# hrnr/map-merge

Hardware: NVIDIA B200
Metric: pairwise_registrations_per_sec (higher is better)
Workload: dtype f32

## Files before the change

map-merge_b200/csrc/icp.cu:

```cuda
#include <algorithm>
#include <cmath>
#include <cstring>
#include <type_traits>

#include "mm3d_internal.cuh"

namespace mm3d {

namespace {

constexpr int IB = 128;
constexpr int NSUM = 17;

struct IcpState {
  float final_t[16];
  float step[16];
  double prev_mse;
  int iterations;
  int active;
  int converged;
  int pad;
};

struct IcpJob {
  GridView tgt;
  ReachView reach;
  const float4* src;
  int ns;
  float4* work;
  long long* sums;
  IcpState* st;
  int* ticket;
  int* next_tile;
  int n_tiles;
  float t0[16];
  long long* sums_log;
  int* nn_slot;
};

struct IcpLoop {
  int n_active;
  int pad[3];
};

struct ReachJob {
  GridView g;
  ReachView r;
  unsigned char* a;
  unsigned char* b;
};

__global__ void __launch_bounds__(256) reach_mark_kernel(const ReachJob* __restrict__ jobs)
{
  const ReachJob& j = jobs[blockIdx.y];
  for (int i = blockIdx.x * blockDim.x + threadIdx.x; i < j.g.n; i += gridDim.x * blockDim.x) {
    const float4 p = j.g.pts[i];
    const int x = floor_to_int(p.x * j.g.inv_leaf) - j.g.min_b[0] - j.r.org[0];
    const int y = floor_to_int(p.y * j.g.inv_leaf) - j.g.min_b[1] - j.r.org[1];
    const int z = floor_to_int(p.z * j.g.inv_leaf) - j.g.min_b[2] - j.r.org[2];
    if (x >= 0 && y >= 0 && z >= 0 && x < j.r.dim[0] && y < j.r.dim[1] && z < j.r.dim[2])
      j.a[((size_t)z * j.r.dim[1] + y) * j.r.dim[0] + x] = 0;
  }
}

__global__ void __launch_bounds__(256) reach_pass_kernel(const ReachJob* __restrict__ jobs, int axis, int margin, int from_a)
{
// ... 9 lines not shown
    const int len = j.r.dim[axis];
    const long long stride = axis == 0 ? 1 : (axis == 1 ? (long long)j.r.dim[0] : (long long)j.r.dim[0] * j.r.dim[1]);
    const int lo = max(-margin, -pos), hi = min(margin, len - 1 - pos);
    int best = 255;
    for (int d = lo; d <= hi; ++d) {
      const int f = max(abs(d) - 1, 0);
      const int v = (int)in[(long long)c + (long long)d * stride] + f * f;
      best = min(best, v);
    }
    out[c] = (unsigned char)min(best, j.r.none);
  }
}

__device__ __forceinline__ bool reach_lookup(const GridView& g, const ReachView& r, float qx, float qy, float qz, int* lb2)
{
  const int x = floor_to_int(qx * g.inv_leaf) - g.min_b[0] - r.org[0];
  const int y = floor_to_int(qy * g.inv_leaf) - g.min_b[1] - r.org[1];
  const int z = floor_to_int(qz * g.inv_leaf) - g.min_b[2] - r.org[2];
  if (x < 0 || y < 0 || z < 0 || x >= r.dim[0] || y >= r.dim[1] || z >= r.dim[2]) return false;
  *lb2 = (int)__ldg(&r.lb2[((size_t)z * r.dim[1] + y) * r.dim[0] + x]);
  return true;
}

__device__ __forceinline__ bool reach_descend(const ReachView& r, int& x, int& y, int& z, int cur)
{
  for (int step = 0; step < 48 && cur > 0; ++step) {
    int best = cur, bx = x, by = y, bz = z;
#pragma unroll
    for (int t = 0; t < 6; ++t) {
      const int nx = x + (t == 0) - (t == 1), ny = y + (t == 2) - (t == 3), nz = z + (t == 4) - (t == 5);
      if (nx < 0 || ny < 0 || nz < 0 || nx >= r.dim[0] || ny >= r.dim[1] || nz >= r.dim[2]) continue;
      const int v = (int)__ldg(&r.lb2[((size_t)nz * r.dim[1] + ny) * r.dim[0] + nx]);
      if (v < best) {
        best = v;
        bx = nx;
        by = ny;
        bz = nz;
      }
    }
    if (best >= cur) return false;
    cur = best;
    x = bx;
    y = by;
    z = bz;
  }
  return cur == 0;
}

__device__ __forceinline__ float block27_any(const GridView& g, int vx, int vy, int vz, float qx, float qy, float qz)
// ... 62 lines not shown
    for (int k = rs[t]; k < re[t]; ++k) {
      const float4 p = g.pts[k];
      const float d2 = em::dist2_3(qx, qy, qz, p.x, p.y, p.z);
      if ((double)d2 > bound) continue;
      const int oi = g.orig ? g.orig[k] : k;
      if (!found || d2 < best || (d2 == best && oi < best_idx)) {
        found = true;
        best = d2;
        best_idx = oi;
        best_slot = k;
        best_pt = p;
        bestv = d2 * inv2 * 1.0001f + 1e-4f;
      }
    }
  }
  *certain = found && best * inv2 < 0.999f;
  *out_idx = best_idx;
  *out_d2 = best;
  *out_pt = best_pt;
  *out_slot = found ? best_slot : -1;
  return found;
}

struct TileNn {
  float4 q[IB];
  int todo[IB];
  int todo_large[IB];
  float res_d2[IB];
  int res_slot[IB];
  int n_todo, n_todo_large;
};

__device__ __forceinline__ bool tile_nearest(TileNn& sh, const GridView& g, const ReachView& r, bool live, float qx, float qy, float qz,
                                             double bound, int guess_slot, float* out_d2, float4* out_pt, int* out_slot)
{
  const int tid = threadIdx.x, lane = tid & 31, warp = tid >> 5;
  if (tid == 0) {
    sh.n_todo = 0;
    sh.n_todo_large = 0;
  }
  __syncthreads();
  bool hit = false, pending = false;
  float d2 = 0.f;
  int slot = -1;
  float4 pt = make_float4(0.f, 0.f, 0.f, 0.f);
  if (live) {
    float r2 = (float)bound;
    bool rejected = false, block_has_points = true;
    if (r.lb2) {
      int lb2 = 0;
      const float bound_v = (float)bound * g.inv_leaf * g.inv_leaf;
      const bool inside = reach_lookup(g, r, qx, qy, qz, &lb2);
      const float lb = inside ? (float)lb2 : (float)r.none;
      if (lb > bound_v * 1.001f + 0.01f) rejected = true;
      if (inside && lb2 < r.none) {
        const float ub = sqrtf((float)lb2) + 3.4642f;
        r2 = fminf(r2, (ub * ub * 1.001f + 0.01f) * g.leaf * g.leaf);
      }
      block_has_points = inside && lb2 == 0;
      if (!rejected && inside && lb2 > 0 && lb2 < r.none && guess_slot < 0 && g.shift[0] == 0 && g.shift[1] == 0 && g.shift[2] == 0) {
        int cx = floor_to_int(qx * g.inv_leaf) - g.min_b[0] - r.org[0];
        int cy = floor_to_int(qy * g.inv_leaf) - g.min_b[1] - r.org[1];
        int cz = floor_to_int(qz * g.inv_leaf) - g.min_b[2] - r.org[2];
        if (reach_descend(r, cx, cy, cz, lb2)) {
          const float dd = block27_any(g, cx + r.org[0], cy + r.org[1], cz + r.org[2], qx, qy, qz);
          if (dd < 3.0e38f) r2 = fminf(r2, dd);
        }
      }
    }
    if (!rejected) {
      bool certain = false;
      if ((block_has_points || guess_slot >= 0) && g.shift[0] == 0 && g.shift[1] == 0 && g.shift[2] == 0) {
        int idx;
        hit = nearest_block27(g, qx, qy, qz, bound, guess_slot, &idx, &d2, &pt, &slot, &certain);
        if (hit) r2 = fminf(r2, d2);
      }
      if (!certain) {
        pending = true;
        hit = false;
        const float r2w = r2 * 1.00001f + 1e-12f;
        sh.q[tid] = make_float4(qx, qy, qz, r2w);
        if (r2w * g.inv_leaf * g.inv_leaf <= 12.25f) sh.todo[atomicAdd(&sh.n_todo, 1)] = tid;
        else sh.todo_large[atomicAdd(&sh.n_todo_large, 1)] = tid;
      }
    }
  }
  __syncthreads();
  const int n_small = sh.n_todo, n_large = sh.n_todo_large;
  auto serve = [&](auto G_, int who, unsigned gmask, int glane) {
    constexpr int G = decltype(G_)::value;
    const float4 q = sh.q[who];
    const int rv = (int)ceilf(sqrtf(q.w) * g.inv_leaf) + 1;
    float bd = 3.0e38f;
    int bi = 0x7fffffff, bs = -1;
    group_radius_unordered<G>(g, gmask, glane, q.x, q.y, q.z, q.w, rv, [&](bool valid, int k, const float4&, float dd) {
      if (valid && (double)dd <= bound) {
        const int oi = g.orig ? g.orig[k] : k;
        if (dd < bd || (dd == bd && oi < bi)) {
          bd = dd;
          bi = oi;
          bs = k;
        }
      }
    });
#pragma unroll
    for (int o = G / 2; o > 0; o >>= 1) {
      const float od = __shfl_xor_sync(gmask, bd, o, G);
      const int oi = __shfl_xor_sync(gmask, bi, o, G);
      const int os = __shfl_xor_sync(gmask, bs, o, G);
      if (od < bd || (od == bd && oi < bi)) {
        bd = od;
        bi = oi;
        bs = os;
      }
    }
    if (glane == 0) {
      sh.res_d2[who] = bd;
      sh.res_slot[who] = bs;
    }
  };
  {
    const int grp = tid >> 3, glane = tid & 7;
    const unsigned gmask = 0xffu << (lane & 24);
    for (int t = grp; t < n_small; t += IB / 8) serve(std::integral_constant<int, 8>(), sh.todo[t], gmask, glane);
  }
  __syncwarp();
  for (int t = warp; t < n_large; t += IB / 32) serve(std::integral_constant<int, 32>(), sh.todo_large[t], 0xffffffffu, lane);
  __syncthreads();
  if (pending) {
    slot = sh.res_slot[tid];
    hit = slot >= 0;
    if (hit) {
      d2 = sh.res_d2[tid];
      pt = g.pts[slot];
    }
  }
  *out_d2 = d2;
  *out_pt = pt;
  *out_slot = hit ? slot : -1;
  return hit;
}

__global__ void __launch_bounds__(256) icp_init_kernel(const IcpJob* __restrict__ jobs)
{
  const IcpJob& j = jobs[blockIdx.y];
  for (int i = blockIdx.x * blockDim.x + threadIdx.x; i < j.ns; i += gridDim.x * blockDim.x) {
    const float4 p = j.src[i];
    float4 o;
    em::transform_point(j.t0, p.x, p.y, p.z, &o.x, &o.y, &o.z);
    o.w = p.w;
    j.work[i] = o;
    j.nn_slot[i] = -1;
  }
}

__device__ __forceinline__ void block_accumulate(long long* vals, int nvals, long long* gsums)
{
  __shared__ long long sh[IB / 32][NSUM];
  const int lane = threadIdx.x & 31, w = threadIdx.x >> 5;
  __syncthreads();
  for (int k = 0; k < nvals; ++k) {
    const long long v = warp_sum_ll(vals[k]);
    if (lane == 0) sh[w][k] = v;
  }
  __syncthreads();
  if (threadIdx.x < nvals) {
    long long s = 0;
    for (int ww = 0; ww < IB / 32; ++ww) s += sh[ww][threadIdx.x];
    if (s != 0) atomicAdd((unsigned long long*)&gsums[threadIdx.x], (unsigned long long)s);
  }
}

__device__ void mat4_mul(const float* a, const float* b, float* r)
{
  for (int i = 0; i < 4; ++i)
    for (int c = 0; c < 4; ++c) {
      float acc = a[i * 4 + 0] * b[0 * 4 + c];
      acc += a[i * 4 + 1] * b[1 * 4 + c];
      acc += a[i * 4 + 2] * b[2 * 4 + c];
      acc += a[i * 4 + 3] * b[3 * 4 + c];
      r[i * 4 + c] = acc;
    }
}

__device__ void icp_solve(const IcpJob& j, int max_iterations, double rotation_threshold, double translation_threshold, int max_log,
                          int* n_active)
{
  IcpState& st = *j.st;
  long long s[NSUM];
  for (int k = 0; k < NSUM; ++k) {
    s[k] = (long long)atomicExch((unsigned long long*)&j.sums[k], 0ull);
  }
  if (j.sums_log && st.iterations < max_log)
// ... 27 lines not shown
    st.step[k] = T[k];
  }
  st.iterations += 1;
  bool conv = false;
  if (st.iterations >= max_iterations) {
    conv = true;
  } else {
    const double cos_angle = 0.5 * (double)(T[0] + T[5] + T[10] - 1);
    const double translation_sqr = (double)(T[3] * T[3] + T[7] * T[7] + T[11] * T[11]);
    if (cos_angle >= rotation_threshold && translation_sqr <= translation_threshold) {
      conv = true;
    } else {
      const double mse = ((double)s[16] / MM3D_FIXD_SCALE) / n;
      if (fabs(mse - st.prev_mse) < 1e-12) conv = true;
      else st.prev_mse = mse;
    }
  }
  if (conv) {
    st.active = 0;
    st.converged = 1;
    __threadfence();
    atomicSub(n_active, 1);
  } else {
    __threadfence();
    atomicExch(j.next_tile, 0);
  }
}

__device__ __forceinline__ void icp_tile(const IcpJob& j, int tile, double max_dist_sqr, int rv, int max_iterations,
                                         double rotation_threshold, double translation_threshold, int max_log, int* n_active)
{
  __shared__ float s_step[16];
  __shared__ int s_apply;
  __shared__ TileNn nn;
  __syncthreads();
  if (threadIdx.x < 16) s_step[threadIdx.x] = __ldcg(&j.st->step[threadIdx.x]);
  if (threadIdx.x == 16) s_apply = __ldcg(&j.st->iterations) > 0 ? 1 : 0;
  __syncthreads();
  const int apply_step = s_apply;
  long long v[NSUM];
#pragma unroll
  for (int k = 0; k < NSUM; ++k) v[k] = 0;
  const int i = tile * IB + threadIdx.x;
  const bool live = i < j.ns;
  float4 p = make_float4(0.f, 0.f, 0.f, 0.f);
  int guess = -1;
  if (live) {
    p = __ldcg(&j.work[i]);
    if (apply_step) {
      float4 o;
      em::transform_point(s_step, p.x, p.y, p.z, &o.x, &o.y, &o.z);
      o.w = p.w;
      p = o;
      j.work[i] = p;
    }
    guess = __ldcg(&j.nn_slot[i]);
  }
  float d2;
  float4 q;
  int slot;
  const bool hit = tile_nearest(nn, j.tgt, j.reach, live, p.x, p.y, p.z, max_dist_sqr, guess, &d2, &q, &slot);
  if (live) {
    j.nn_slot[i] = slot;
    if (hit) {
      const double pp[3] = {(double)p.x, (double)p.y, (double)p.z};
      const double qq[3] = {(double)q.x, (double)q.y, (double)q.z};
      v[0] = 1;
#pragma unroll
      for (int a = 0; a < 3; ++a) {
        v[1 + a] = em::to_fix(pp[a], MM3D_FIX1_SCALE);
        v[4 + a] = em::to_fix(qq[a], MM3D_FIX1_SCALE);
#pragma unroll
        for (int b = 0; b < 3; ++b) v[7 + a * 3 + b] = em::to_fix(qq[a] * pp[b], MM3D_FIX2_SCALE);
      }
      v[16] = em::to_fix((double)d2, MM3D_FIXD_SCALE);
    }
  }
  block_accumulate(v, NSUM, j.sums);
  __syncthreads();
  if (threadIdx.x == 0) {
    __threadfence();
    const int ntiles = (j.ns + IB - 1) / IB;
    const int ticket = atomicAdd(j.ticket, 1);
    if (ticket == ntiles - 1) {
      *j.ticket = 0;
      __threadfence();
      icp_solve(j, max_iterations, rotation_threshold, translation_threshold, max_log, n_active);
    }
  }
}

__global__ void __launch_bounds__(IB) icp_persistent_kernel(const IcpJob* __restrict__ jobs, int n_jobs, IcpLoop* loop, double max_dist_sqr,
                                                            int rv, int max_iterations, double rotation_threshold,
                                                            double translation_threshold, int max_log)
{
  __shared__ int s_pair, s_tile;
  int cur = 0;
  for (;;) {
    if (threadIdx.x == 0) {
      int pair = -1, tile = -1, scanned = 0;
      while (__ldcg(&loop->n_active) > 0) {
        const IcpJob& j = jobs[cur];
        if (__ldcg(j.next_tile) < j.n_tiles) {
          const int t = atomicAdd(j.next_tile, 1);
          if (t < j.n_tiles) {
            __threadfence();
            pair = cur;
            tile = t;
            break;
          }
        }
        cur = cur + 1 == n_jobs ? 0 : cur + 1;
        if (++scanned >= n_jobs) {
          scanned = 0;
          __nanosleep(500);
        }
      }
      s_pair = pair;
      s_tile = tile;
    }
    __syncthreads();
    const int pair = s_pair, tile = s_tile;
    if (pair < 0) break;
    icp_tile(jobs[pair], tile, max_dist_sqr, rv, max_iterations, rotation_threshold, translation_threshold, max_log, &loop->n_active);
    __syncthreads();
  }
}

struct ScoreJob {
  GridView tgt;
  ReachView reach;
  const float4* src;
  int ns;
  float t[16];
  long long* sums;
  const int* nn_guess;
};

__global__ void __launch_bounds__(IB) score_kernel(const ScoreJob* __restrict__ jobs, double max_range, int rv)
{
  const ScoreJob& j = jobs[blockIdx.y];
  if (blockIdx.x * IB >= j.ns) return;
  __shared__ TileNn nn;
  long long v[2] = {0, 0};
  const int i = blockIdx.x * IB + threadIdx.x;
  const bool live = i < j.ns;
  float x = 0.f, y = 0.f, z = 0.f;
  if (live) {
    const float4 p = j.src[i];
    em::transform_point(j.t, p.x, p.y, p.z, &x, &y, &z);
  }
  float d2;
  float4 q;
  int slot;
  if (tile_nearest(nn, j.tgt, j.reach, live, x, y, z, max_range, (live && j.nn_guess) ? j.nn_guess[i] : -1, &d2, &q, &slot)) {
    v[0] = em::to_fix((double)d2, MM3D_FIXD_SCALE);
    v[1] = 1;
  }
  block_accumulate(v, 2, j.sums);
}

ReachView no_reach()
{
  ReachView r;
  memset(&r, 0, sizeof(r));
  return r;
}

}

void build_reach_batch(Ctx& c, const std::vector<DIndex>& idx, int margin, std::vector<DReach>& out)
{
  const int M = (int)idx.size();
  out.clear();
  out.resize(M);
  margin = std::max(2, std::min(margin, 15));
  std::vector<ReachJob> jobs;
  std::vector<DBuf<unsigned char>> ping(M);
  size_t max_cells = 0;
  int max_n = 0;
  for (int m = 0; m < M; ++m) {
    out[m].v = no_reach();
// ... 50 lines not shown
    if (zero) {
      for (int k = 0; k < 16; ++k) out[p].T[k] = 0.0f;
      out[p].iterations = 0;
      out[p].converged = 0;
    } else {
      act.push_back(p);
    }
  }
  const int A = (int)act.size();
  if (A == 0) return;
  std::stable_sort(act.begin(), act.end(), [&](int x, int y) { return jobs[x].b < jobs[y].b; });
  size_t tot = 0;
  int mx = 0;
  for (int a = 0; a < A; ++a) {
    tot += (size_t)clouds[jobs[act[a]].a].n;
    mx = std::max(mx, clouds[jobs[act[a]].a].n);
  }
  DBuf<float4> work(c, tot + 1);
  DBuf<int> nn_local;
  DBuf<int>& nn = nn_keep ? nn_keep->slots : nn_local;
  nn.alloc(c, tot + 1);
  DBuf<long long> sums(c, (size_t)A * NSUM);
  sums.zero(c);
  DBuf<int> tickets(c, A);
  tickets.zero(c);
  DBuf<long long> slog;
  if (max_log) {
    slog.alloc(c, (size_t)A * max_log * NSUM);
    slog.zero(c);
  }
  std::vector<IcpState> hst(A);
  for (int a = 0; a < A; ++a) {
    memset(&hst[a], 0, sizeof(IcpState));
    for (int k = 0; k < 16; ++k) hst[a].final_t[k] = hst[a].step[k] = (k % 5 == 0) ? 1.f : 0.f;
    hst[a].prev_mse = 1.7976931348623157e308;
    hst[a].active = clouds[jobs[act[a]].a].n > 0 ? 1 : 0;
  }
  DBuf<IcpState> dst = to_device(c, hst);
  std::vector<IcpJob> ij(A);
  size_t off = 0;
  for (int a = 0; a < A; ++a) {
    const PairJob& pj = jobs[act[a]];
    ij[a].tgt = idx[pj.b].v;
    ij[a].reach = pj.b < (int)reach.size() ? reach[pj.b].v : no_reach();
    ij[a].src = clouds[pj.a].pts;
    ij[a].ns = clouds[pj.a].n;
    ij[a].work = work.p + off;
    ij[a].nn_slot = nn.p + off;
    if (nn_keep) nn_keep->offset[act[a]] = (long long)off;
    ij[a].sums = sums.p + (size_t)a * NSUM;
    ij[a].st = dst.p + a;
    ij[a].ticket = tickets.p + a;
    for (int k = 0; k < 16; ++k) ij[a].t0[k] = T0[act[a]][k];
    ij[a].sums_log = max_log ? slog.p + (size_t)a * max_log * NSUM : nullptr;
    off += (size_t)ij[a].ns;
  }
  std::vector<int> hnext(A, 0);
  IcpLoop hl;
  memset(&hl, 0, sizeof(hl));
  int tiles = 0;
  double bytes = 0;
  for (int a = 0; a < A; ++a) {
    ij[a].n_tiles = (ij[a].ns + IB - 1) / IB;
    if (hst[a].active) {
      hl.n_active += 1;
      tiles += ij[a].n_tiles;
      bytes += 16.0 * (2.0 * ij[a].ns + ij[a].tgt.n);
    } else {
      hnext[a] = ij[a].n_tiles;
    }
  }
  DBuf<int> dnext = to_device(c, hnext);
  for (int a = 0; a < A; ++a) ij[a].next_tile = dnext.p + a;
  DBuf<IcpJob> dij = to_device(c, ij);
  DBuf<IcpLoop> dloop(c, 1);
  dloop.upload(c, &hl, 1);
  const int iblocks = std::max(1, std::min((mx + 255) / 256, 148 * 8));
  MM_LAUNCH(c, icp_init_kernel, dim3(iblocks, A), 256, 0, dij.p);
  const double max_dist_sqr = max_dist * max_dist;
  const float leaf = idx[jobs[act[0]].b].v.leaf;
  const int rv = (int)std::ceil(max_dist / (double)leaf) + 1;
  if (hl.n_active > 0) {
    int dev = 0, sms = 0, per_sm = 0;
    MM_CUDA(cudaGetDevice(&dev));
    MM_CUDA(cudaDeviceGetAttribute(&sms, cudaDevAttrMultiProcessorCount, dev));
    MM_CUDA(cudaOccupancyMaxActiveBlocksPerMultiprocessor(&per_sm, icp_persistent_kernel, IB, 0));
    const int grid = std::max(1, std::min(sms * std::max(per_sm, 1), tiles));
    MM_BYTES(c, bytes);
    MM_LAUNCH(c, icp_persistent_kernel, grid, IB, 0, dij.p, A, dloop.p, max_dist_sqr, rv, max_it, 1.0 - eps, eps, max_log);
  }
  dst.download(c, hst.data(), A);
  std::vector<long long> hlog;
  if (max_log) {
    hlog.resize((size_t)A * max_log * NSUM);
    slog.download(c, hlog.data(), hlog.size());
  }
  c.sync();
  for (int a = 0; a < A; ++a) {
    IcpOut& o = out[act[a]];
    const float* f = hst[a].final_t;
    const float* g = T0[act[a]];
    for (int i = 0; i < 4; ++i)
      for (int cc = 0; cc < 4; ++cc) {
        float acc = f[i * 4 + 0] * g[0 * 4 + cc];
        acc += f[i * 4 + 1] * g[1 * 4 + cc];
        acc += f[i * 4 + 2] * g[2 * 4 + cc];
        acc += f[i * 4 + 3] * g[3 * 4 + cc];
        o.T[i * 4 + cc] = acc;
      }
    o.iterations = hst[a].iterations;
    o.converged = hst[a].converged;
    if (sums_dbg) {
      const int nl = std::min(hst[a].iterations + (hst[a].converged ? 0 : 1), max_log);
      (*sums_dbg)[act[a]].assign(hlog.begin() + (size_t)a * max_log * NSUM, hlog.begin() + ((size_t)a * max_log + nl) * NSUM);
    }
  }
}

void score_batch(Ctx& c, const std::vector<CloudView>& clouds, const std::vector<DIndex>& idx, const std::vector<DReach>& reach,
                 const std::vector<PairJob>& jobs, const std::vector<const float*>& T, double max_range, std::vector<double>& scores,
                 const IcpNeighbours* nn_guess)
{
  const int P = (int)jobs.size();
  scores.assign(P, 1.7976931348623157e308);
  if (P == 0) return;
  DBuf<long long> sums(c, (size_t)P * 2);
  sums.zero(c);
  std::vector<ScoreJob> sj(P);
  int mx = 0;
  std::vector<int> ord(P);
  for (int p = 0; p < P; ++p) ord[p] = p;
  std::stable_sort(ord.begin(), ord.end(), [&](int x, int y) { return jobs[x].b < jobs[y].b; });
  for (int q = 0; q < P; ++q) {
    const int p = ord[q];
    sj[q].tgt = idx[jobs[p].b].v;
    sj[q].reach = jobs[p].b < (int)reach.size() ? reach[jobs[p].b].v : no_reach();
    sj[q].src = clouds[jobs[p].a].pts;
    sj[q].ns = clouds[jobs[p].a].n;
    for (int k = 0; k < 16; ++k) sj[q].t[k] = T[p][k];
    sj[q].sums = sums.p + (size_t)p * 2;
    sj[q].nn_guess = (nn_guess && p < (int)nn_guess->offset.size() && nn_guess->offset[p] >= 0) ? nn_guess->slots.p + nn_guess->offset[p] : nullptr;
    mx = std::max(mx, sj[q].ns);
  }
  if (mx == 0) return;
  DBuf<ScoreJob> dsj = to_device(c, sj);
  const float leaf = idx[jobs[0].b].v.leaf;
  const int rv = (int)std::ceil(std::sqrt(std::max(max_range, 0.0)) / (double)leaf) + 1;
  { double b = 0; for (int p = 0; p < P; ++p) b += 16.0 * ((double)sj[p].ns + sj[p].tgt.n); MM_BYTES(c, b); }
  MM_LAUNCH(c, score_kernel, dim3((mx + IB - 1) / IB, P), IB, 0, dsj.p, max_range, rv);
  std::vector<long long> h((size_t)P * 2);
  sums.download(c, h.data(), h.size());
  c.sync();
  for (int p = 0; p < P; ++p)
    if (h[2 * p + 1] > 0) scores[p] = ((double)h[2 * p] / MM3D_FIXD_SCALE) / (double)h[2 * p + 1];
}

}
```

Measured before the change: 1062.

## Defer uncertain nearest-neighbour queries to compacted far-query batches with row-parallel search

Tile-local nearest-neighbour search no longer serves the uncertain queries inside each tile. Those far queries now go into global queues with per-job pending counters and are served in compacted batches. A new far_nearest routine spreads grid rows across a lane group, uses prefix-sum load balancing over candidates and shrinks the search radius as it goes. Scoring gets the same treatment through a separate score_far_kernel, and an optional counters build plus a profiling script are added. The aim is to cut load imbalance and idle lanes when only a few queries per tile miss the fast path. The cost is extra global traffic, atomics, an added kernel launch and more complex completion tracking.

```diff
diff --git a/map-merge_b200/csrc/icp.cu b/map-merge_b200/csrc/icp.cu
--- a/map-merge_b200/csrc/icp.cu
+++ b/map-merge_b200/csrc/icp.cu
@@ -30,8 +30,12 @@
   float4* work;
   long long* sums;
   IcpState* st;
-  int* ticket;
+  int* pending;
   int* next_tile;
+  int* tiles_left;
+  float4* far_q;
+  int* far_tag;
+  unsigned long long* far_ctr;
   int n_tiles;
   float t0[16];
   long long* sums_log;
@@ -42,6 +46,22 @@
   int n_active;
   int pad[3];
 };
+
+constexpr int CTR_SETS = 9;
+#ifdef MM3D_ICP_COUNTERS
+constexpr int CTR_ROW_BINS = 1024, CTR_FAR_BINS = IB + 1;
+enum { C_QUERIES, C_REJECTED, C_SETTLED, C_SMALL, C_LARGE, C_ROWS_SMALL, C_ROWS_LARGE, C_CAND_SMALL, C_CAND_LARGE, C_DESCENDS,
+       C_DESCEND_STEPS, C_TILES, C_N = 16 };
+struct CtrSet {
+  unsigned long long c[C_N];
+  unsigned long long rows_small[CTR_ROW_BINS], rows_large[CTR_ROW_BINS];
+  unsigned long long far_per_tile[CTR_FAR_BINS];
+};
+__device__ CtrSet g_ctr[CTR_SETS];
+#define ICP_CTR(...) __VA_ARGS__
+#else
+#define ICP_CTR(...)
+#endif
 
 struct ReachJob {
   GridView g;
@@ -97,9 +117,10 @@
   return true;
 }
 
-__device__ __forceinline__ bool reach_descend(const ReachView& r, int& x, int& y, int& z, int cur)
+__device__ __forceinline__ bool reach_descend(const ReachView& r, int& x, int& y, int& z, int cur, int& steps)
 {
   for (int step = 0; step < 48 && cur > 0; ++step) {
+    steps = step + 1;
     int best = cur, bx = x, by = y, bz = z;
 #pragma unroll
     for (int t = 0; t < 6; ++t) {
@@ -208,28 +229,52 @@
   return found;
 }
 
-struct TileNn {
-  float4 q[IB];
-  int todo[IB];
-  int todo_large[IB];
-  float res_d2[IB];
-  int res_slot[IB];
-  int n_todo, n_todo_large;
-};
-
-__device__ __forceinline__ bool tile_nearest(TileNn& sh, const GridView& g, const ReachView& r, bool live, float qx, float qy, float qz,
-                                             double bound, int guess_slot, float* out_d2, float4* out_pt, int* out_slot)
-{
-  const int tid = threadIdx.x, lane = tid & 31, warp = tid >> 5;
-  if (tid == 0) {
-    sh.n_todo = 0;
-    sh.n_todo_large = 0;
-  }
-  __syncthreads();
-  bool hit = false, pending = false;
-  float d2 = 0.f;
-  int slot = -1;
-  float4 pt = make_float4(0.f, 0.f, 0.f, 0.f);
+enum NearResult { NEAR_NONE, NEAR_HIT, NEAR_FAR };
+
+#ifdef MM3D_ICP_COUNTERS
+__device__ void ctr_window(const GridView& g, float qx, float qy, float qz, float r2, int rv, int* rows, int* cands)
+{
+  *rows = 0;
+  *cands = 0;
+  const int vx = floor_to_int(qx * g.inv_leaf) - g.min_b[0];
+  const int vy = floor_to_int(qy * g.inv_leaf) - g.min_b[1];
+  const int vz = floor_to_int(qz * g.inv_leaf) - g.min_b[2];
+  int zlo = vz - rv, zhi = vz + rv, ylo = vy - rv, yhi = vy + rv;
+  if (zhi < 0 || yhi < 0 || vx + rv < 0 || zlo >= g.div_v[2] || ylo >= g.div_v[1] || vx - rv >= g.div_v[0]) return;
+  zlo = max(zlo, 0) >> g.shift[2];
+  zhi = min(zhi, g.div_v[2] - 1) >> g.shift[2];
+  ylo = max(ylo, 0) >> g.shift[1];
+  yhi = min(yhi, g.div_v[1] - 1) >> g.shift[1];
+  *rows = (zhi - zlo + 1) * (yhi - ylo + 1);
+  const float r2v = r2 * g.inv_leaf * g.inv_leaf;
+  for (int cz = zlo; cz <= zhi; ++cz)
+    for (int cy = ylo; cy <= yhi; ++cy) {
+      const int z0 = cz << g.shift[2], z1 = z0 + (1 << g.shift[2]) - 1;
+      const int y0 = cy << g.shift[1], y1 = y0 + (1 << g.shift[1]) - 1;
+      const float fz = (float)max(max(max(z0 - vz, vz - z1), 0) - 1, 0);
+      const float fy = (float)max(max(max(y0 - vy, vy - y1), 0) - 1, 0);
+      const float rem = r2v - fz * fz - fy * fy;
+      if (rem < 0.0f) continue;
+      const int rx = (int)sqrtf(rem) + 2;
+      int xlo = vx - rx, xhi = vx + rx;
+      if (xhi < 0 || xlo >= g.div_v[0]) continue;
+      xlo = max(xlo, 0) >> g.shift[0];
+      xhi = min(xhi, g.div_v[0] - 1) >> g.shift[0];
+      const int base = (cz * g.dim[1] + cy) * g.dim[0];
+      *cands += g.cell_start[base + xhi + 1] - g.cell_start[base + xlo];
+    }
+}
+#endif
+
+__device__ __forceinline__ NearResult query_near(const GridView& g, const ReachView& r, bool live, float qx, float qy, float qz,
+                                                 double bound, int guess_slot, float* out_d2, float4* out_pt, int* out_slot,
+                                                 float* far_r2, int ctr_set)
+{
+  (void)ctr_set;
+  ICP_CTR(CtrSet& cs = g_ctr[ctr_set]);
+  ICP_CTR(if (live) atomicAdd(&cs.c[C_QUERIES], 1ull));
+  ICP_CTR(if (threadIdx.x == 0) atomicAdd(&cs.c[C_TILES], 1ull));
+  NearResult res = NEAR_NONE;
   if (live) {
     float r2 = (float)bound;
     bool rejected = false, block_has_points = true;
@@ -248,83 +293,204 @@
         int cx = floor_to_int(qx * g.inv_leaf) - g.min_b[0] - r.org[0];
         int cy = floor_to_int(qy * g.inv_leaf) - g.min_b[1] - r.org[1];
         int cz = floor_to_int(qz * g.inv_leaf) - g.min_b[2] - r.org[2];
-        if (reach_descend(r, cx, cy, cz, lb2)) {
+        int steps = 0;
+        const bool down = reach_descend(r, cx, cy, cz, lb2, steps);
+        ICP_CTR(atomicAdd(&cs.c[C_DESCENDS], 1ull); atomicAdd(&cs.c[C_DESCEND_STEPS], (unsigned long long)steps));
+        if (down) {
           const float dd = block27_any(g, cx + r.org[0], cy + r.org[1], cz + r.org[2], qx, qy, qz);
           if (dd < 3.0e38f) r2 = fminf(r2, dd);
         }
       }
     }
+    ICP_CTR(if (rejected) atomicAdd(&cs.c[C_REJECTED], 1ull));
     if (!rejected) {
-      bool certain = false;
+      bool certain = false, hit = false;
       if ((block_has_points || guess_slot >= 0) && g.shift[0] == 0 && g.shift[1] == 0 && g.shift[2] == 0) {
         int idx;
-        hit = nearest_block27(g, qx, qy, qz, bound, guess_slot, &idx, &d2, &pt, &slot, &certain);
-        if (hit) r2 = fminf(r2, d2);
+        hit = nearest_block27(g, qx, qy, qz, bound, guess_slot, &idx, out_d2, out_pt, out_slot, &certain);
+        if (hit) r2 = fminf(r2, *out_d2);
       }
-      if (!certain) {
-        pending = true;
-        hit = false;
-        const float r2w = r2 * 1.00001f + 1e-12f;
-        sh.q[tid] = make_float4(qx, qy, qz, r2w);
-        if (r2w * g.inv_leaf * g.inv_leaf <= 12.25f) sh.todo[atomicAdd(&sh.n_todo, 1)] = tid;
-        else sh.todo_large[atomicAdd(&sh.n_todo_large, 1)] = tid;
+      ICP_CTR(if (certain) atomicAdd(&cs.c[C_SETTLED], 1ull));
+      if (certain) {
+        res = NEAR_HIT;
+      } else {
+        res = NEAR_FAR;
+        *far_r2 = r2 * 1.00001f + 1e-12f;
+#ifdef MM3D_ICP_COUNTERS
+        const bool small = *far_r2 * g.inv_leaf * g.inv_leaf <= 12.25f;
+        int rows, cands;
+        ctr_window(g, qx, qy, qz, *far_r2, (int)ceilf(sqrtf(*far_r2) * g.inv_leaf) + 1, &rows, &cands);
+        atomicAdd(&cs.c[small ? C_SMALL : C_LARGE], 1ull);
+        atomicAdd(&cs.c[small ? C_ROWS_SMALL : C_ROWS_LARGE], (unsigned long long)rows);
+        atomicAdd(&cs.c[small ? C_CAND_SMALL : C_CAND_LARGE], (unsigned long long)cands);
+        atomicAdd(small ? &cs.rows_small[min(rows, CTR_ROW_BINS - 1)] : &cs.rows_large[min(rows, CTR_ROW_BINS - 1)], 1ull);
+#endif
       }
     }
   }
-  __syncthreads();
-  const int n_small = sh.n_todo, n_large = sh.n_todo_large;
-  auto serve = [&](auto G_, int who, unsigned gmask, int glane) {
-    constexpr int G = decltype(G_)::value;
-    const float4 q = sh.q[who];
-    const int rv = (int)ceilf(sqrtf(q.w) * g.inv_leaf) + 1;
-    float bd = 3.0e38f;
-    int bi = 0x7fffffff, bs = -1;
-    group_radius_unordered<G>(g, gmask, glane, q.x, q.y, q.z, q.w, rv, [&](bool valid, int k, const float4&, float dd) {
-      if (valid && (double)dd <= bound) {
-        const int oi = g.orig ? g.orig[k] : k;
-        if (dd < bd || (dd == bd && oi < bi)) {
-          bd = dd;
-          bi = oi;
-          bs = k;
+#ifdef MM3D_ICP_COUNTERS
+  const int n_far = __syncthreads_count(res == NEAR_FAR);
+  if (threadIdx.x == 0) atomicAdd(&cs.far_per_tile[n_far], 1ull);
+#endif
+  return res;
+}
+
+template <int G>
+__device__ __forceinline__ void far_nearest(const GridView& g, unsigned gmask, int glane, const float4& q, double bound, float* out_d2,
+                                            int* out_slot)
+{
+  constexpr int R = 4;
+  float bd = 3.0e38f;
+  int bi = 0x7fffffff, bs = -1;
+  const int rv = (int)ceilf(sqrtf(q.w) * g.inv_leaf) + 1;
+  const int vx = floor_to_int(q.x * g.inv_leaf) - g.min_b[0];
+  const int vy = floor_to_int(q.y * g.inv_leaf) - g.min_b[1];
+  const int vz = floor_to_int(q.z * g.inv_leaf) - g.min_b[2];
+  int zlo = vz - rv, zhi = vz + rv, ylo = vy - rv, yhi = vy + rv;
+  if (!(zhi < 0 || yhi < 0 || vx + rv < 0 || zlo >= g.div_v[2] || ylo >= g.div_v[1] || vx - rv >= g.div_v[0])) {
+    zlo = max(zlo, 0) >> g.shift[2];
+    zhi = min(zhi, g.div_v[2] - 1) >> g.shift[2];
+    ylo = max(ylo, 0) >> g.shift[1];
+    yhi = min(yhi, g.div_v[1] - 1) >> g.shift[1];
+    const int ny = yhi - ylo + 1;
+    const int n_rows = (zhi - zlo + 1) * ny;
+    const unsigned ny_magic = 0xFFFFFFFFu / (unsigned)ny + 1u;
+    float r2 = q.w;
+    for (int row0 = 0; row0 < n_rows; row0 += G * R) {
+      const float r2v = r2 * g.inv_leaf * g.inv_leaf;
+      int s[R], e[R];
+#pragma unroll
+      for (int r = 0; r < R; ++r) {
+        s[r] = 0;
+        e[r] = 0;
+        const int row = row0 + r * G + glane;
+        if (row < n_rows) {
+          const int rq = (int)__umulhi((unsigned)row, ny_magic);
+          const int cz = zlo + rq, cy = ylo + (row - rq * ny);
+          const int z0 = cz << g.shift[2], z1 = z0 + (1 << g.shift[2]) - 1;
+          const int y0 = cy << g.shift[1], y1 = y0 + (1 << g.shift[1]) - 1;
+          const float fz = (float)max(max(max(z0 - vz, vz - z1), 0) - 1, 0);
+          const float fy = (float)max(max(max(y0 - vy, vy - y1), 0) - 1, 0);
+          const float rem = r2v - fz * fz - fy * fy;
+          if (rem >= 0.0f) {
+            const int rx = (int)sqrtf(rem) + 2;
+            int xlo = vx - rx, xhi = vx + rx;
+            if (xhi >= 0 && xlo < g.div_v[0]) {
+              xlo = max(xlo, 0) >> g.shift[0];
+              xhi = min(xhi, g.div_v[0] - 1) >> g.shift[0];
+              const int base = (cz * g.dim[1] + cy) * g.dim[0];
+              s[r] = __ldg(&g.cell_start[base + xlo]);
+              e[r] = __ldg(&g.cell_start[base + xhi + 1]);
+            }
+          }
         }
       }
-    });
-#pragma unroll
-    for (int o = G / 2; o > 0; o >>= 1) {
-      const float od = __shfl_xor_sync(gmask, bd, o, G);
-      const int oi = __shfl_xor_sync(gmask, bi, o, G);
-      const int os = __shfl_xor_sync(gmask, bs, o, G);
-      if (od < bd || (od == bd && oi < bi)) {
-        bd = od;
-        bi = oi;
-        bs = os;
+#pragma unroll
+      for (int r = 0; r < R; ++r) {
+        int incl = e[r] - s[r];
+#pragma unroll
+        for (int o = 1; o < G; o <<= 1) {
+          const int t = __shfl_up_sync(gmask, incl, o, G);
+          if (glane >= o) incl += t;
+        }
+        const int total = __shfl_sync(gmask, incl, G - 1, G);
+        const int excl = incl - (e[r] - s[r]);
+        for (int t0 = 0; t0 < total; t0 += G) {
+          const int t = t0 + glane;
+          int L = 0;
+#pragma unroll
+          for (int step = G / 2; step >= 1; step >>= 1) {
+            const int v = __shfl_sync(gmask, incl, L + step - 1, G);
+            if (v <= t) L += step;
+          }
+          L = min(L, G - 1);
+          const int ls = __shfl_sync(gmask, s[r], L, G), le = __shfl_sync(gmask, excl, L, G);
+          if (t < total) {
+            const int k = ls + (t - le);
+            const float4 p = g.pts[k];
+            const float dd = em::dist2_3(q.x, q.y, q.z, p.x, p.y, p.z);
+            if (dd < r2 && (double)dd <= bound) {
+              const int oi = g.orig ? g.orig[k] : k;
+              if (dd < bd || (dd == bd && oi < bi)) {
+                bd = dd;
+                bi = oi;
+                bs = k;
+              }
+            }
+          }
+        }
       }
-    }
-    if (glane == 0) {
-      sh.res_d2[who] = bd;
-      sh.res_slot[who] = bs;
-    }
-  };
+      float m = bd;
+#pragma unroll
+      for (int o = G / 2; o > 0; o >>= 1) m = fminf(m, __shfl_xor_sync(gmask, m, o, G));
+      if (m < 3.0e38f) r2 = fminf(r2, m * 1.00001f + 1e-12f);
+    }
+  }
+#pragma unroll
+  for (int o = G / 2; o > 0; o >>= 1) {
+    const float od = __shfl_xor_sync(gmask, bd, o, G);
+    const int oi = __shfl_xor_sync(gmask, bi, o, G);
+    const int os = __shfl_xor_sync(gmask, bs, o, G);
+    if (od < bd || (od == bd && oi < bi)) {
+      bd = od;
+      bi = oi;
+      bs = os;
+    }
+  }
+  *out_d2 = bd;
+  *out_slot = bs;
+}
+
+constexpr int FB = IB / 8;
+struct FarBatch {
+  float4 q[FB];
+  int who[FB];
+  int small[FB], large[FB];
+  int n_small, n_large;
+  float res_d2[FB];
+  int res_slot[FB];
+};
+
+template <typename GridOf>
+__device__ __forceinline__ void serve_far(FarBatch& sh, int n, double bound, GridOf grid)
+{
+  const int tid = threadIdx.x, lane = tid & 31, warp = tid >> 5;
+  if (tid == 0) {
+    int ns = 0, nl = 0;
+    for (int t = 0; t < n; ++t) {
+      if (sh.q[t].w * grid(t).inv_leaf * grid(t).inv_leaf <= 12.25f) sh.small[ns++] = t;
+      else sh.large[nl++] = t;
+    }
+    sh.n_small = ns;
+    sh.n_large = nl;
+  }
+  __syncthreads();
+  const int n_small = sh.n_small, n_large = sh.n_large;
   {
     const int grp = tid >> 3, glane = tid & 7;
     const unsigned gmask = 0xffu << (lane & 24);
-    for (int t = grp; t < n_small; t += IB / 8) serve(std::integral_constant<int, 8>(), sh.todo[t], gmask, glane);
+    for (int t = grp; t < n_small; t += IB / 8) {
+      const int e = sh.small[t];
+      float d2;
+      int slot;
+      far_nearest<8>(grid(e), gmask, glane, sh.q[e], bound, &d2, &slot);
+      if (glane == 0) {
+        sh.res_d2[e] = d2;
+        sh.res_slot[e] = slot;
+      }
+    }
   }
   __syncwarp();
-  for (int t = warp; t < n_large; t += IB / 32) serve(std::integral_constant<int, 32>(), sh.todo_large[t], 0xffffffffu, lane);
-  __syncthreads();
-  if (pending) {
-    slot = sh.res_slot[tid];
-    hit = slot >= 0;
-    if (hit) {
-      d2 = sh.res_d2[tid];
-      pt = g.pts[slot];
-    }
-  }
-  *out_d2 = d2;
-  *out_pt = pt;
-  *out_slot = hit ? slot : -1;
-  return hit;
+  for (int t = warp; t < n_large; t += IB / 32) {
+    const int e = sh.large[t];
+    float d2;
+    int slot;
+    far_nearest<32>(grid(e), 0xffffffffu, lane, sh.q[e], bound, &d2, &slot);
+    if (lane == 0) {
+      sh.res_d2[e] = d2;
+      sh.res_slot[e] = slot;
+    }
+  }
 }
 
 __global__ void __launch_bounds__(256) icp_init_kernel(const IcpJob* __restrict__ jobs)
@@ -355,6 +521,21 @@
     for (int ww = 0; ww < IB / 32; ++ww) s += sh[ww][threadIdx.x];
     if (s != 0) atomicAdd((unsigned long long*)&gsums[threadIdx.x], (unsigned long long)s);
   }
+}
+
+__device__ __forceinline__ void icp_terms(const float4& p, const float4& q, float d2, long long* v)
+{
+  const double pp[3] = {(double)p.x, (double)p.y, (double)p.z};
+  const double qq[3] = {(double)q.x, (double)q.y, (double)q.z};
+  v[0] = 1;
+#pragma unroll
+  for (int a = 0; a < 3; ++a) {
+    v[1 + a] = em::to_fix(pp[a], MM3D_FIX1_SCALE);
+    v[4 + a] = em::to_fix(qq[a], MM3D_FIX1_SCALE);
+#pragma unroll
+    for (int b = 0; b < 3; ++b) v[7 + a * 3 + b] = em::to_fix(qq[a] * pp[b], MM3D_FIX2_SCALE);
+  }
+  v[16] = em::to_fix((double)d2, MM3D_FIXD_SCALE);
 }
 
 __device__ void mat4_mul(const float* a, const float* b, float* r)
@@ -428,22 +609,34 @@
     __threadfence();
     atomicSub(n_active, 1);
   } else {
+    *j.pending = j.n_tiles;
+    *j.tiles_left = j.n_tiles;
+    *j.far_ctr = 0ull;
     __threadfence();
     atomicExch(j.next_tile, 0);
   }
 }
 
-__device__ __forceinline__ void icp_tile(const IcpJob& j, int tile, double max_dist_sqr, int rv, int max_iterations,
-                                         double rotation_threshold, double translation_threshold, int max_log, int* n_active)
+__device__ __forceinline__ void icp_retire(const IcpJob& j, int units, int max_iterations, double rotation_threshold,
+                                           double translation_threshold, int max_log, int* n_active)
+{
+  __threadfence();
+  if (atomicSub(j.pending, units) == units) {
+    __threadfence();
+    icp_solve(j, max_iterations, rotation_threshold, translation_threshold, max_log, n_active);
+  }
+}
+
+__device__ __forceinline__ void icp_tile(const IcpJob& j, int tile, double max_dist_sqr, int max_iterations, double rotation_threshold,
+                                         double translation_threshold, int max_log, int* n_active)
 {
   __shared__ float s_step[16];
-  __shared__ int s_apply;
-  __shared__ TileNn nn;
+  __shared__ int s_iter;
   __syncthreads();
   if (threadIdx.x < 16) s_step[threadIdx.x] = __ldcg(&j.st->step[threadIdx.x]);
-  if (threadIdx.x == 16) s_apply = __ldcg(&j.st->iterations) > 0 ? 1 : 0;
+  if (threadIdx.x == 16) s_iter = __ldcg(&j.st->iterations);
   __syncthreads();
-  const int apply_step = s_apply;
+  const int iter = s_iter;
   long long v[NSUM];
 #pragma unroll
   for (int k = 0; k < NSUM; ++k) v[k] = 0;
@@ -453,7 +646,7 @@
   int guess = -1;
   if (live) {
     p = __ldcg(&j.work[i]);
-    if (apply_step) {
+    if (iter > 0) {
       float4 o;
       em::transform_point(s_step, p.x, p.y, p.z, &o.x, &o.y, &o.z);
       o.w = p.w;
@@ -462,51 +655,102 @@
     }
     guess = __ldcg(&j.nn_slot[i]);
   }
-  float d2;
-  float4 q;
-  int slot;
-  const bool hit = tile_nearest(nn, j.tgt, j.reach, live, p.x, p.y, p.z, max_dist_sqr, guess, &d2, &q, &slot);
-  if (live) {
+  float d2 = 0.f, far_r2 = 0.f;
+  float4 q = make_float4(0.f, 0.f, 0.f, 0.f);
+  int slot = -1;
+  const NearResult nr = query_near(j.tgt, j.reach, live, p.x, p.y, p.z, max_dist_sqr, guess, &d2, &q, &slot, &far_r2,
+                                   min(iter, CTR_SETS - 2));
+  const int lane = threadIdx.x & 31;
+  const unsigned far_mask = __ballot_sync(0xffffffffu, nr == NEAR_FAR);
+  if (far_mask) {
+    unsigned base = 0;
+    if (lane == 0) {
+      atomicAdd(j.pending, __popc(far_mask));
+      __threadfence();
+      base = (unsigned)atomicAdd(j.far_ctr, (unsigned long long)__popc(far_mask));
+    }
+    base = __shfl_sync(0xffffffffu, base, 0);
+    if (nr == NEAR_FAR) {
+      const unsigned e = base + __popc(far_mask & ((1u << lane) - 1u));
+      __stcg(&j.far_q[e], make_float4(p.x, p.y, p.z, far_r2));
+      __threadfence();
+      atomicExch(&j.far_tag[e], i + 1);
+    }
+  }
+  if (live && nr != NEAR_FAR) {
     j.nn_slot[i] = slot;
-    if (hit) {
-      const double pp[3] = {(double)p.x, (double)p.y, (double)p.z};
-      const double qq[3] = {(double)q.x, (double)q.y, (double)q.z};
-      v[0] = 1;
-#pragma unroll
-      for (int a = 0; a < 3; ++a) {
-        v[1 + a] = em::to_fix(pp[a], MM3D_FIX1_SCALE);
-        v[4 + a] = em::to_fix(qq[a], MM3D_FIX1_SCALE);
-#pragma unroll
-        for (int b = 0; b < 3; ++b) v[7 + a * 3 + b] = em::to_fix(qq[a] * pp[b], MM3D_FIX2_SCALE);
-      }
-      v[16] = em::to_fix((double)d2, MM3D_FIXD_SCALE);
-    }
+    if (nr == NEAR_HIT) icp_terms(p, q, d2, v);
   }
   block_accumulate(v, NSUM, j.sums);
   __syncthreads();
   if (threadIdx.x == 0) {
     __threadfence();
-    const int ntiles = (j.ns + IB - 1) / IB;
-    const int ticket = atomicAdd(j.ticket, 1);
-    if (ticket == ntiles - 1) {
-      *j.ticket = 0;
-      __threadfence();
-      icp_solve(j, max_iterations, rotation_threshold, translation_threshold, max_log, n_active);
-    }
-  }
-}
-
-__global__ void __launch_bounds__(IB) icp_persistent_kernel(const IcpJob* __restrict__ jobs, int n_jobs, IcpLoop* loop, double max_dist_sqr,
-                                                            int rv, int max_iterations, double rotation_threshold,
-                                                            double translation_threshold, int max_log)
-{
-  __shared__ int s_pair, s_tile;
+    atomicSub(j.tiles_left, 1);
+    icp_retire(j, 1, max_iterations, rotation_threshold, translation_threshold, max_log, n_active);
+  }
+}
+
+__device__ __forceinline__ bool far_claim(unsigned long long* ctr, int min_n, int* base, int* n)
+{
+  unsigned long long w = __ldcg(ctr);
+  for (;;) {
+    const int reserved = (int)(unsigned)w, claimed = (int)(w >> 32);
+    const int k = min(reserved - claimed, FB);
+    if (k < min_n) return false;
+    const unsigned long long o = atomicCAS(ctr, w, w + ((unsigned long long)k << 32));
+    if (o == w) {
+      *base = claimed;
+      *n = k;
+      return true;
+    }
+    w = o;
+  }
+}
+
+__device__ __forceinline__ void icp_far(const IcpJob& j, int base, int n, double max_dist_sqr, int max_iterations, double rotation_threshold,
+                                        double translation_threshold, int max_log, int* n_active)
+{
+  __shared__ FarBatch fb;
+  __syncthreads();
+  if (threadIdx.x < n) {
+    const int e = base + threadIdx.x;
+    int tag;
+    while ((tag = __ldcg(&j.far_tag[e])) == 0) __nanosleep(20);
+    fb.who[threadIdx.x] = tag - 1;
+    fb.q[threadIdx.x] = __ldcg(&j.far_q[e]);
+    __stcg(&j.far_tag[e], 0);
+  }
+  __syncthreads();
+  serve_far(fb, n, max_dist_sqr, [&](int) -> const GridView& { return j.tgt; });
+  __syncthreads();
+  long long v[NSUM];
+#pragma unroll
+  for (int k = 0; k < NSUM; ++k) v[k] = 0;
+  if (threadIdx.x < n) {
+    const int t = threadIdx.x, slot = fb.res_slot[t];
+    j.nn_slot[fb.who[t]] = slot;
+    if (slot >= 0) icp_terms(fb.q[t], j.tgt.pts[slot], fb.res_d2[t], v);
+  }
+  block_accumulate(v, NSUM, j.sums);
+  __syncthreads();
+  if (threadIdx.x == 0) icp_retire(j, n, max_iterations, rotation_threshold, translation_threshold, max_log, n_active);
+}
+
+__global__ void __launch_bounds__(IB, 8) icp_persistent_kernel(const IcpJob* __restrict__ jobs, int n_jobs, IcpLoop* loop, double max_dist_sqr,
+                                                            int max_iterations, double rotation_threshold, double translation_threshold,
+                                                            int max_log)
+{
+  __shared__ int s_pair, s_tile, s_base, s_n;
   int cur = 0;
   for (;;) {
     if (threadIdx.x == 0) {
-      int pair = -1, tile = -1, scanned = 0;
+      int pair = -1, tile = -1, base = 0, n = 0, scanned = 0;
       while (__ldcg(&loop->n_active) > 0) {
         const IcpJob& j = jobs[cur];
+        if (far_claim(j.far_ctr, FB, &base, &n)) {
+          pair = cur;
+          break;
+        }
         if (__ldcg(j.next_tile) < j.n_tiles) {
           const int t = atomicAdd(j.next_tile, 1);
           if (t < j.n_tiles) {
@@ -516,6 +760,10 @@
             break;
           }
         }
+        if (__ldcg(j.tiles_left) == 0 && far_claim(j.far_ctr, 1, &base, &n)) {
+          pair = cur;
+          break;
+        }
         cur = cur + 1 == n_jobs ? 0 : cur + 1;
         if (++scanned >= n_jobs) {
           scanned = 0;
@@ -524,11 +772,14 @@
       }
       s_pair = pair;
       s_tile = tile;
+      s_base = base;
+      s_n = n;
     }
     __syncthreads();
-    const int pair = s_pair, tile = s_tile;
+    const int pair = s_pair, tile = s_tile, base = s_base, n = s_n;
     if (pair < 0) break;
-    icp_tile(jobs[pair], tile, max_dist_sqr, rv, max_iterations, rotation_threshold, translation_threshold, max_log, &loop->n_active);
+    if (tile >= 0) icp_tile(jobs[pair], tile, max_dist_sqr, max_iterations, rotation_threshold, translation_threshold, max_log, &loop->n_active);
+    else icp_far(jobs[pair], base, n, max_dist_sqr, max_iterations, rotation_threshold, translation_threshold, max_log, &loop->n_active);
     __syncthreads();
   }
 }
@@ -543,11 +794,11 @@
   const int* nn_guess;
 };
 
-__global__ void __launch_bounds__(IB) score_kernel(const ScoreJob* __restrict__ jobs, double max_range, int rv)
+__global__ void __launch_bounds__(IB) score_kernel(const ScoreJob* __restrict__ jobs, double max_range, float4* __restrict__ far_q,
+                                                   int* __restrict__ far_job, unsigned* far_ctr)
 {
   const ScoreJob& j = jobs[blockIdx.y];
   if (blockIdx.x * IB >= j.ns) return;
-  __shared__ TileNn nn;
   long long v[2] = {0, 0};
   const int i = blockIdx.x * IB + threadIdx.x;
   const bool live = i < j.ns;
@@ -556,14 +807,68 @@
     const float4 p = j.src[i];
     em::transform_point(j.t, p.x, p.y, p.z, &x, &y, &z);
   }
-  float d2;
+  float d2 = 0.f, far_r2 = 0.f;
   float4 q;
   int slot;
-  if (tile_nearest(nn, j.tgt, j.reach, live, x, y, z, max_range, (live && j.nn_guess) ? j.nn_guess[i] : -1, &d2, &q, &slot)) {
+  const NearResult nr = query_near(j.tgt, j.reach, live, x, y, z, max_range, (live && j.nn_guess) ? j.nn_guess[i] : -1, &d2, &q, &slot,
+                                   &far_r2, CTR_SETS - 1);
+  if (nr == NEAR_HIT) {
     v[0] = em::to_fix((double)d2, MM3D_FIXD_SCALE);
     v[1] = 1;
   }
+  const int lane = threadIdx.x & 31;
+  const unsigned far_mask = __ballot_sync(0xffffffffu, nr == NEAR_FAR);
+  if (far_mask) {
+    unsigned base = 0;
+    if (lane == 0) base = atomicAdd(far_ctr, (unsigned)__popc(far_mask));
+    base = __shfl_sync(0xffffffffu, base, 0);
+    if (nr == NEAR_FAR) {
+      const unsigned e = base + __popc(far_mask & ((1u << lane) - 1u));
+      far_q[e] = make_float4(x, y, z, far_r2);
+      far_job[e] = blockIdx.y;
+    }
+  }
   block_accumulate(v, 2, j.sums);
+}
+
+__global__ void __launch_bounds__(IB) score_far_kernel(const ScoreJob* __restrict__ jobs, double max_range, const float4* __restrict__ far_q,
+                                                       const int* __restrict__ far_job, unsigned* far_ctr)
+{
+  __shared__ FarBatch fb;
+  __shared__ int s_base;
+  const int total = (int)far_ctr[0];
+  for (;;) {
+    __syncthreads();
+    if (threadIdx.x == 0) s_base = (int)atomicAdd(&far_ctr[1], (unsigned)FB);
+    __syncthreads();
+    const int base = s_base;
+    if (base >= total) break;
+    const int n = min(FB, total - base);
+    if (threadIdx.x < n) {
+      fb.q[threadIdx.x] = far_q[base + threadIdx.x];
+      fb.who[threadIdx.x] = far_job[base + threadIdx.x];
+    }
+    __syncthreads();
+    serve_far(fb, n, max_range, [&](int t) -> const GridView& { return jobs[fb.who[t]].tgt; });
+    __syncthreads();
+    if (threadIdx.x == 0) {
+      long long sd = 0, nr = 0;
+      for (int t = 0; t < n; ++t) {
+        if (fb.res_slot[t] >= 0) {
+          sd += em::to_fix((double)fb.res_d2[t], MM3D_FIXD_SCALE);
+          nr += 1;
+        }
+        if (t + 1 == n || fb.who[t + 1] != fb.who[t]) {
+          long long* s = jobs[fb.who[t]].sums;
+          if (nr) {
+            atomicAdd((unsigned long long*)&s[0], (unsigned long long)sd);
+            atomicAdd((unsigned long long*)&s[1], (unsigned long long)nr);
+          }
+          sd = nr = 0;
+        }
+      }
+    }
+  }
 }
 
 ReachView no_reach()
@@ -660,8 +965,11 @@
   nn.alloc(c, tot + 1);
   DBuf<long long> sums(c, (size_t)A * NSUM);
   sums.zero(c);
-  DBuf<int> tickets(c, A);
-  tickets.zero(c);
+  DBuf<float4> far_q(c, tot + 1);
+  DBuf<int> far_tag(c, tot + 1);
+  far_tag.zero(c);
+  DBuf<unsigned long long> far_ctr(c, A);
+  far_ctr.zero(c);
   DBuf<long long> slog;
   if (max_log) {
     slog.alloc(c, (size_t)A * max_log * NSUM);
@@ -688,18 +996,21 @@
     if (nn_keep) nn_keep->offset[act[a]] = (long long)off;
     ij[a].sums = sums.p + (size_t)a * NSUM;
     ij[a].st = dst.p + a;
-    ij[a].ticket = tickets.p + a;
+    ij[a].far_q = far_q.p + off;
+    ij[a].far_tag = far_tag.p + off;
+    ij[a].far_ctr = far_ctr.p + a;
     for (int k = 0; k < 16; ++k) ij[a].t0[k] = T0[act[a]][k];
     ij[a].sums_log = max_log ? slog.p + (size_t)a * max_log * NSUM : nullptr;
     off += (size_t)ij[a].ns;
   }
-  std::vector<int> hnext(A, 0);
+  std::vector<int> hnext(A, 0), hpending(A, 0);
   IcpLoop hl;
   memset(&hl, 0, sizeof(hl));
   int tiles = 0;
   double bytes = 0;
   for (int a = 0; a < A; ++a) {
     ij[a].n_tiles = (ij[a].ns + IB - 1) / IB;
+    hpending[a] = ij[a].n_tiles;
     if (hst[a].active) {
       hl.n_active += 1;
       tiles += ij[a].n_tiles;
@@ -708,16 +1019,18 @@
       hnext[a] = ij[a].n_tiles;
     }
   }
-  DBuf<int> dnext = to_device(c, hnext);
-  for (int a = 0; a < A; ++a) ij[a].next_tile = dnext.p + a;
+  DBuf<int> dnext = to_device(c, hnext), dpending = to_device(c, hpending), dtiles_left = to_device(c, hpending);
+  for (int a = 0; a < A; ++a) {
+    ij[a].next_tile = dnext.p + a;
+    ij[a].pending = dpending.p + a;
+    ij[a].tiles_left = dtiles_left.p + a;
+  }
   DBuf<IcpJob> dij = to_device(c, ij);
   DBuf<IcpLoop> dloop(c, 1);
   dloop.upload(c, &hl, 1);
   const int iblocks = std::max(1, std::min((mx + 255) / 256, 148 * 8));
   MM_LAUNCH(c, icp_init_kernel, dim3(iblocks, A), 256, 0, dij.p);
   const double max_dist_sqr = max_dist * max_dist;
-  const float leaf = idx[jobs[act[0]].b].v.leaf;
-  const int rv = (int)std::ceil(max_dist / (double)leaf) + 1;
   if (hl.n_active > 0) {
     int dev = 0, sms = 0, per_sm = 0;
     MM_CUDA(cudaGetDevice(&dev));
@@ -725,7 +1038,7 @@
     MM_CUDA(cudaOccupancyMaxActiveBlocksPerMultiprocessor(&per_sm, icp_persistent_kernel, IB, 0));
     const int grid = std::max(1, std::min(sms * std::max(per_sm, 1), tiles));
     MM_BYTES(c, bytes);
-    MM_LAUNCH(c, icp_persistent_kernel, grid, IB, 0, dij.p, A, dloop.p, max_dist_sqr, rv, max_it, 1.0 - eps, eps, max_log);
+    MM_LAUNCH(c, icp_persistent_kernel, grid, IB, 0, dij.p, A, dloop.p, max_dist_sqr, max_it, 1.0 - eps, eps, max_log);
   }
   dst.download(c, hst.data(), A);
   std::vector<long long> hlog;
@@ -766,6 +1079,7 @@
   sums.zero(c);
   std::vector<ScoreJob> sj(P);
   int mx = 0;
+  size_t tot = 0;
   std::vector<int> ord(P);
   for (int p = 0; p < P; ++p) ord[p] = p;
   std::stable_sort(ord.begin(), ord.end(), [&](int x, int y) { return jobs[x].b < jobs[y].b; });
@@ -779,13 +1093,21 @@
     sj[q].sums = sums.p + (size_t)p * 2;
     sj[q].nn_guess = (nn_guess && p < (int)nn_guess->offset.size() && nn_guess->offset[p] >= 0) ? nn_guess->slots.p + nn_guess->offset[p] : nullptr;
     mx = std::max(mx, sj[q].ns);
+    tot += (size_t)sj[q].ns;
   }
   if (mx == 0) return;
   DBuf<ScoreJob> dsj = to_device(c, sj);
-  const float leaf = idx[jobs[0].b].v.leaf;
-  const int rv = (int)std::ceil(std::sqrt(std::max(max_range, 0.0)) / (double)leaf) + 1;
+  DBuf<float4> far_q(c, tot);
+  DBuf<int> far_job(c, tot);
+  DBuf<unsigned> far_ctr(c, 2);
+  far_ctr.zero(c);
   { double b = 0; for (int p = 0; p < P; ++p) b += 16.0 * ((double)sj[p].ns + sj[p].tgt.n); MM_BYTES(c, b); }
-  MM_LAUNCH(c, score_kernel, dim3((mx + IB - 1) / IB, P), IB, 0, dsj.p, max_range, rv);
+  MM_LAUNCH(c, score_kernel, dim3((mx + IB - 1) / IB, P), IB, 0, dsj.p, max_range, far_q.p, far_job.p, far_ctr.p);
+  int dev = 0, sms = 0, per_sm = 0;
+  MM_CUDA(cudaGetDevice(&dev));
+  MM_CUDA(cudaDeviceGetAttribute(&sms, cudaDevAttrMultiProcessorCount, dev));
+  MM_CUDA(cudaOccupancyMaxActiveBlocksPerMultiprocessor(&per_sm, score_far_kernel, IB, 0));
+  MM_LAUNCH(c, score_far_kernel, sms * std::max(per_sm, 1), IB, 0, dsj.p, max_range, far_q.p, far_job.p, far_ctr.p);
   std::vector<long long> h((size_t)P * 2);
   sums.download(c, h.data(), h.size());
   c.sync();
@@ -794,3 +1116,16 @@
 }
 
 }
+
+#ifdef MM3D_ICP_COUNTERS
+extern "C" int mm3d_icp_counters(unsigned long long* out, int n, int reset)
+{
+  const int words = (int)(sizeof(mm3d::g_ctr) / 8);
+  if (out && n >= words && cudaMemcpyFromSymbol(out, mm3d::g_ctr, sizeof(mm3d::g_ctr)) != cudaSuccess) return -1;
+  if (reset) {
+    static const mm3d::CtrSet zero[mm3d::CTR_SETS] = {};
+    if (cudaMemcpyToSymbol(mm3d::g_ctr, zero, sizeof(zero)) != cudaSuccess) return -1;
+  }
+  return words;
+}
+#endif
diff --git a/profiles/icp_query_classes.py b/profiles/icp_query_classes.py
--- /dev/null
+++ b/profiles/icp_query_classes.py
@@ -0,0 +1,135 @@
+import argparse
+import ctypes as C
+import glob
+import json
+import os
+import subprocess
+import sys
+import tempfile
+from concurrent.futures import ThreadPoolExecutor
+
+import numpy as np
+
+ROOT = os.path.dirname(os.path.dirname(os.path.abspath(__file__)))
+PKG = os.path.join(ROOT, "map-merge_b200")
+sys.path.insert(0, ROOT)
+
+NAMES = ["queries", "rejected", "settled_block27", "small_windows", "large_windows", "rows_small", "rows_large", "cand_small",
+         "cand_large", "descends", "descend_steps", "tiles"]
+C_N, ROW_BINS, FAR_BINS, SETS = 16, 1024, 129, 9
+SET_WORDS = C_N + 2 * ROW_BINS + FAR_BINS
+
+
+def card():
+    q = subprocess.run(["nvidia-smi", "--query-gpu=name,power.limit", "--format=csv,noheader"], capture_output=True, text=True)
+    first = q.stdout.strip().splitlines()[0] if q.returncode == 0 and q.stdout.strip() else ""
+    name, _, power = first.partition(",")
+    return {"name": name.strip() or None, "power_limit": power.strip() or None}
+
+
+def build_counters_lib(tmp):
+    arch = ["-gencode", "arch=compute_100a,code=sm_100a"]
+    flags = [*arch, "-O3", "-std=c++17", "-lineinfo", "-fmad=false", "-Xcompiler", "-fPIC,-ffp-contract=off"]
+    srcs = sorted(glob.glob(os.path.join(PKG, "csrc", "*.cu"))) + [os.path.join(PKG, "csrc", "graph.cpp")]
+
+    def compile_one(src):
+        obj = os.path.join(tmp, os.path.basename(src) + ".o")
+        extra = ["-DMM3D_ICP_COUNTERS"] if os.path.basename(src) == "icp.cu" else []
+        subprocess.check_call(["nvcc", *flags, *extra, "-x", "cu", "-c", src, "-o", obj])
+        return obj
+
+    with ThreadPoolExecutor(max_workers=os.cpu_count() or 4) as ex:
+        objs = list(ex.map(compile_one, srcs))
+    lib = os.path.join(tmp, "libmm3d.so")
+    subprocess.check_call(["nvcc", *arch, "-shared", "-o", lib, *objs, "-lcudart", "-ldl"])
+    return lib
+
+
+def p99(hist):
+    tot = hist.sum()
+    if tot == 0:
+        return None
+    return int(np.searchsorted(np.cumsum(hist), 0.99 * tot))
+
+
+def summarise(words):
+    c = {n: int(words[k]) for k, n in enumerate(NAMES)}
+    rows_small = words[C_N:C_N + ROW_BINS]
+    rows_large = words[C_N + ROW_BINS:C_N + 2 * ROW_BINS]
+    far = words[C_N + 2 * ROW_BINS:SET_WORDS]
+    win = c["small_windows"] + c["large_windows"]
+    out = dict(c)
+    out["far_queries"] = win
+    out["far_share"] = win / c["queries"] if c["queries"] else None
+    for kind, h in (("small", rows_small), ("large", rows_large)):
+        n = c[f"{kind}_windows"]
+        out[f"rows_per_{kind}_window_mean"] = c[f"rows_{kind}"] / n if n else None
+        out[f"rows_per_{kind}_window_p99"] = p99(h)
+        out[f"cand_per_{kind}_window_mean"] = c[f"cand_{kind}"] / n if n else None
+    out["rows_per_window_p99"] = p99(rows_small + rows_large)
+    out["cand_per_query_mean"] = (c["cand_small"] + c["cand_large"]) / c["queries"] if c["queries"] else None
+    out["steps_per_descend_mean"] = c["descend_steps"] / c["descends"] if c["descends"] else None
+    out["far_per_tile_hist"] = {str(k): int(v) for k, v in enumerate(far) if v}
+    tiles = int(far.sum())
+    out["tiles_with_far_queries"] = tiles - int(far[0])
+    out["far_per_tile_mean"] = float((np.arange(FAR_BINS) * far).sum() / tiles) if tiles else None
+    return out
+
+
+def dumps(res):
+    lines = []
+    for k, v in res.items():
+        if k == "icp":
+            inner = ",\n".join(f"  {json.dumps(n)}: {json.dumps(s)}" for n, s in v.items())
+            lines.append(f" {json.dumps(k)}: {{\n{inner}\n }}")
+        else:
+            lines.append(f" {json.dumps(k)}: {json.dumps(v)}")
+    return "{\n" + ",\n".join(lines) + "\n}\n"
+
+
+def main():
+    ap = argparse.ArgumentParser()
+    ap.add_argument("--out", required=True)
+    args = ap.parse_args()
+    import mm3d_pkg
+    mm = mm3d_pkg.load()
+    synth = mm3d_pkg.load_synth()
+    with tempfile.TemporaryDirectory() as tmp:
+        mm.LIB_PATH = build_counters_lib(tmp)
+        L = mm.lib()
+        L.mm3d_icp_counters.restype = C.c_int
+        L.mm3d_icp_counters.argtypes = [C.POINTER(C.c_ulonglong), C.c_int, C.c_int]
+        words = L.mm3d_icp_counters(None, 0, 0)
+        assert words == SETS * SET_WORDS, (words, SETS * SET_WORDS)
+        ctx = mm.Context(0)
+        maps, _ = synth.make_maps(**synth.CONFIGS["c3"])
+        params = mm.default_params(descriptor_type="FPFH")
+        ctx.estimate_maps_transforms(maps, params)
+        L.mm3d_icp_counters(None, 0, 1)
+        ctx.estimate_maps_transforms(maps, params)
+        buf = np.zeros(words, np.uint64)
+        assert L.mm3d_icp_counters(buf.ctypes.data_as(C.POINTER(C.c_ulonglong)), words, 1) == words
+        ctx.close()
+    sets = buf.reshape(SETS, SET_WORDS)
+    res = {"card": card(), "workload": "c3: 32 maps x 1M points, SIFT + FPFH, 496 pairs",
+           "max_correspondence_distance": params.max_correspondence_distance, "resolution": params.resolution,
+           "icp": {}, "score": summarise(sets[SETS - 1])}
+    for k in range(SETS - 1):
+        s = summarise(sets[k])
+        if s["queries"]:
+            res["icp"][f"iteration_{k}" + ("_and_later" if k == SETS - 2 else "")] = s
+    tot = sets[:SETS - 1].sum(axis=0)
+    res["icp_all_iterations"] = summarise(tot)
+    os.makedirs(os.path.dirname(os.path.abspath(args.out)), exist_ok=True)
+    with open(args.out, "w") as f:
+        f.write(dumps(res))
+    brief = {k: res[k] for k in ("card",)}
+    for name, s in (("icp", res["icp_all_iterations"]), ("score", res["score"])):
+        brief[name] = {k: s[k] for k in ("queries", "rejected", "settled_block27", "small_windows", "large_windows", "far_share",
+                                         "rows_per_window_p99", "cand_per_query_mean", "steps_per_descend_mean",
+                                         "tiles", "tiles_with_far_queries", "far_per_tile_mean")}
+    print(json.dumps(brief, indent=1))
+
+
+if __name__ == "__main__":
+    main()
```

After: 397.3, median of 6. -62.6%, worse.
